# pinellolab/GRAFIMO

Hardware: AMD Instinct MI355X
Metric: scored haplotype k-mers/sec (higher is better)
Workload: dtype int32

## Files before the change

grafimo_amd/csrc/gfm_score_kernels.hpp:

```cpp
#pragma once

#include "gfm_common.hpp"

namespace {

constexpr int kWave = 64;
constexpr int kThreads = 1024;
constexpr int kWavesPerWG = kThreads / kWave;
constexpr unsigned kPoison = 0xFFFFu;
constexpr int kMaxLdsBytes = 160 * 1024;
constexpr int kWGsPerCU = 1;
constexpr int kReserveCUs = 4;
constexpr int kHitQueue = 64;

constexpr int kWorkspaces = GFM_WORKSPACE_RING;
constexpr int kCtlSlots = 2 * GFM_WORKSPACE_RING;
constexpr int kCtlAhead = GFM_WORKSPACE_RING;
struct HitCtl {
    unsigned long long mid[kCtlSlots];
    unsigned long long snap[kCtlSlots];
};
constexpr int kResidPerWG = kWavesPerWG * kHitQueue;

__device__ inline void hitq_push(long long *hitq, int &qn, bool hit, long long entry, int lane,
// ... 7 lines not shown
        unsigned long long base = 0;
        if (lane == 0) base = (hit_count ? *hit_count : 0ull) + atomicAdd(mid, (unsigned long long)qn);
        base = __shfl(base, 0);
        for (int i = lane; i < qn; i += kWave)
            if ((long long)(base + i) < hit_cap) hit_rows[base + i] = hitq[i];
        qn = 0;
    }
    if (hit) hitq[qn + __popcll(mask & ((1ull << lane) - 1ull))] = entry;
    qn += nh;
}

template <int WAVES>
__device__ inline void hitq_finish(const long long *hitq, int qn, int *wq_n ,
                                   int wave, int lane, int tid, long long *resid, int *resid_n)
{
    if (lane == 0) wq_n[wave] = qn;
    __syncthreads();
    int base = 0, tot = 0;
#pragma unroll
    for (int w = 0; w < WAVES; ++w) {
        if (w < wave) base += wq_n[w];
        tot += wq_n[w];
    }
    long long *slab = resid + (size_t)blockIdx.x * kResidPerWG;
    for (int i = lane; i < qn; i += kWave) slab[base + i] = hitq[i];
    if (tid == 0) resid_n[blockIdx.x] = tot;
}

constexpr int kSpillCopies = 16;

struct MotifArgs {
    const uint16_t *tab;
    int lo, nb, min_val;
    int use_hist;
    int spill_lo;
    int spill_n;
    unsigned *spill;
    int cutoff;
    int slot;
    int *scores;
    unsigned *partials;
    long long *hit_rows;
    long long hit_cap;
    const unsigned long long *hit_count;
    HitCtl *ctl;
    long long *resid;
    int *resid_n;
};
template <int MM> struct ScoreArgs {
    MotifArgs m[MM];
    int store_through;
};

typedef __attribute__((address_space(3))) const unsigned lds_cu32;
typedef __attribute__((address_space(3))) const uint16_t lds_cu16;
typedef __attribute__((address_space(3))) const unsigned long long lds_cu64;
__device__ inline unsigned lds_offset(const void *p)
{
    return (unsigned)(size_t)(__attribute__((address_space(3))) const char *)p;
}

constexpr int kSlabsPerGroup = 16;
constexpr int kPostJobs = 3;
struct PostJob {
    const unsigned *partials;
    unsigned long long *hist64;
    unsigned *spill;
    const long long *resid;
    const int *resid_n;
    HitCtl *ctl;
    long long *hit_rows;
    unsigned long long *hit_count;
    long long hit_cap;
    int nslabs, nb, lo, min_val, bin_blocks, hist_blocks, spill_lo, spill_n, spill_blocks, hit_slabs, par, total;
};
struct PostJobs { PostJob j[kPostJobs]; };

__device__ inline void
post_body(const unsigned *__restrict__ partials, int nslabs, int nb, int lo, int min_val,
          unsigned long long *__restrict__ hist64, int bin_blocks, int hist_blocks,
          unsigned *__restrict__ spill, int spill_lo, int spill_n, int spill_blocks,
          const long long *__restrict__ resid, const int *__restrict__ resid_n, int hit_slabs,
          HitCtl *__restrict__ ctl, int par, long long *__restrict__ hit_rows, long long hit_cap,
          unsigned long long *__restrict__ hit_count)
{
    const int tid = threadIdx.x;
    if (blockIdx.x == 0 && tid == 0 && hit_slabs == 0 && ctl) ctl->mid[(par + kCtlAhead) % kCtlSlots] = 0ull;
    if ((int)blockIdx.x < hist_blocks) {
        const int bx = blockIdx.x % bin_blocks, by = blockIdx.x / bin_blocks;
        const int b = bx * 256 + tid;
        if (b > nb) return;
        const int g0 = by * kSlabsPerGroup;
        const int g1 = min(g0 + kSlabsPerGroup, nslabs);
        unsigned long long s = 0;
        const size_t stride = (size_t)(nb + 1);
#pragma unroll 8
        for (int g = g0; g < g1; ++g) s += __builtin_nontemporal_load(&partials[g * stride + b]);
        if (s) atomicAdd(&hist64[b == nb ? min_val : lo + b], s);
        return;
    }
    if ((int)blockIdx.x < hist_blocks + spill_blocks) {
        const int b = ((int)blockIdx.x - hist_blocks) * 256 + tid;
        if (b < spill_n) {
            unsigned long long v = 0;
#pragma unroll
            for (int c = 0; c < kSpillCopies; ++c) {
                const unsigned x = spill[(size_t)c * (size_t)spill_n + b];
                if (x) {
                    v += x;
                    spill[(size_t)c * (size_t)spill_n + b] = 0u;
                }
            }
            if (v) atomicAdd(&hist64[spill_lo + b], v);
        }
        return;
    }
    __shared__ int part[256];
    __shared__ int part_all[256];
    const int g = blockIdx.x - hist_blocks - spill_blocks;
    int s = 0, sa = 0;
    for (int k = tid; k < hit_slabs; k += 256) {
        const int v = resid_n[k];
        sa += v;
        if (k < g) s += v;
    }
    part[tid] = s;
    part_all[tid] = sa;
    __syncthreads();
    for (int d = 128; d > 0; d >>= 1) {
        if (tid < d) { part[tid] += part[tid + d]; part_all[tid] += part_all[tid + d]; }
        __syncthreads();
    }
    const unsigned long long start = ctl->snap[par] + ctl->mid[par];
    const unsigned long long base = start + (unsigned long long)part[0];
    const int cnt = resid_n[g];
    const long long *slab = resid + (size_t)g * kResidPerWG;
    for (int i = tid; i < cnt; i += 256)
        if ((long long)(base + i) < hit_cap) __builtin_nontemporal_store(__builtin_nontemporal_load(&slab[i]), &hit_rows[base + i]);
    if (g == 0 && tid == 0) {
        *hit_count = start + (unsigned long long)part_all[0];
        ctl->mid[(par + kCtlAhead) % kCtlSlots] = 0ull;
    }
}

__global__ void __launch_bounds__(256) post_kernel(const PostJobs jobs)
{
    const PostJob &q = jobs.j[blockIdx.y];
    if ((int)blockIdx.x >= q.total) return;
    post_body(q.partials, q.nslabs, q.nb, q.lo, q.min_val, q.hist64, q.bin_blocks, q.hist_blocks, q.spill, q.spill_lo,
              q.spill_n, q.spill_blocks, q.resid, q.resid_n, q.hit_slabs, q.ctl, q.par, q.hit_rows, q.hit_cap,
              q.hit_count);
}

constexpr int kSelThreads = 256;
__global__ void __launch_bounds__(kSelThreads)
select_hits_kernel(const int *__restrict__ scores, long long n, const int *__restrict__ cutoff_ptr,
                   long long row_base, long long *__restrict__ hit_rows, long long hit_cap,
                   const unsigned long long *__restrict__ hit_count, HitCtl *__restrict__ ctl,
                   int par, long long *__restrict__ resid, int *__restrict__ resid_n,
                   const unsigned long long *__restrict__ gate_count, long long gate_cap)
{
    __shared__ long long hq[kSelThreads / kWave][kHitQueue];
    __shared__ int wq_n[kSelThreads / kWave];
    const int cutoff = *cutoff_ptr;
    const int tid = threadIdx.x, lane = tid & 63, wave = tid >> 6;
    long long *hitq = hq[wave];
    int qn = 0;
    if (gate_count) {
        if ((long long)*gate_count <= gate_cap) {
            if (tid == 0) {
                resid_n[blockIdx.x] = 0;
                if (blockIdx.x == 0) ctl->snap[par] = hit_count ? *hit_count : 0ull;
            }
            return;
        }
        hit_count = nullptr;
    }
    if (blockIdx.x == 0 && tid == 0) ctl->snap[par] = hit_count ? *hit_count : 0ull;
    const long long nthreads = (long long)gridDim.x * blockDim.x;
    const long long n4 = (n + 3) >> 2;
    const long long iters = (n4 + nthreads - 1) / nthreads;
    const long long t0 = (long long)blockIdx.x * blockDim.x + tid;
// ... 75 lines not shown
```

grafimo_amd/csrc/gfm_score_quad.hpp:

```cpp
#pragma once

#include "gfm_score_kernels.hpp"
#include "gfm_quad_launch.hpp"

namespace {

typedef unsigned u32x2_t __attribute__((ext_vector_type(2)));
typedef unsigned u32x4_t __attribute__((ext_vector_type(4)));
typedef __attribute__((address_space(3))) const u32x2_t lds_cu32x2;
typedef __attribute__((address_space(3))) const u32x4_t lds_cu32x4;
typedef int i32x4 __attribute__((ext_vector_type(4)));

template <int W, int MM, bool STORE = true>
__global__ void __launch_bounds__(kThreads)
score_quad_kernel(const uint8_t *__restrict__ kmers, long long n, long long row_base, const ScoreArgs<MM> a)
{
    extern __shared__ __attribute__((aligned(16))) unsigned char smem[];
    constexpr int NDW = (W + 3) / 4;
    constexpr int kTabBytes = quad_tab_bytes(W, MM);
    constexpr int CB = kQuadRows * W;
    constexpr int kLoads = (CB + 1023) / 1024;
    constexpr int GP = quad_pitch(W);
    constexpr int PAD = quad_pad(W);
    constexpr int SSTRIDE = quad_strip_stride(W, MM);

    if (lds_offset(smem) != 0u) __builtin_trap();
    const int tid = threadIdx.x;
    const int lane = tid & (kWave - 1);
    const int wave = __builtin_amdgcn_readfirstlane(tid >> 6);
    const int n_waves = (int)(blockDim.x >> 6);
    const int wg_threads = (int)blockDim.x;
    unsigned char *tab = smem;
    unsigned char *stage_base = smem + kTabBytes;
    unsigned *hist[MM];
    {
        unsigned *h = reinterpret_cast<unsigned *>(stage_base + n_waves * SSTRIDE);
#pragma unroll
        for (int m = 0; m < MM; ++m) {
            hist[m] = h;
            if (a.m[m].use_hist) h += a.m[m].nb + 1;
        }
    }

    unsigned char *stage = stage_base + wave * SSTRIDE;
    const unsigned stage_off = (unsigned)(kTabBytes + wave * SSTRIDE);
    const long long nfull = n / kQuadRows;
    const long long cstride = (long long)gridDim.x * n_waves;
    bool vec_store = true;
    const bool through = a.store_through == 1;
    constexpr bool no_store = !STORE;
#pragma unroll
    for (int m = 0; m < MM; ++m) vec_store = vec_store && (reinterpret_cast<uintptr_t>(a.m[m].scores) & 15u) == 0;

    uint4 pre[kQuadDepth][kLoads];
    auto fetch = [&](uint4 (&dst)[kLoads], long long c) {
        const uint8_t *src = kmers + c * (long long)CB + lane * 16;
#pragma unroll
        for (int i = 0; i < kLoads; ++i) {
            if (i * 1024 + 1024 <= CB || i * 1024 + lane * 16 < CB) {
                typedef unsigned u32x4 __attribute__((ext_vector_type(4)));
                const u32x4 t = __builtin_nontemporal_load(reinterpret_cast<const u32x4 *>(src + i * 1024));
                dst[i] = make_uint4(t.x, t.y, t.z, t.w);
            }
        }
    };

    long long *hitq[MM];
    int qn[MM];
    bool select[MM];
#pragma unroll
    for (int m = 0; m < MM; ++m) {
        hitq[m] = reinterpret_cast<long long *>(stage + quad_stage_bytes(W)) + m * kHitQueue;
        qn[m] = 0;
        select[m] = a.m[m].cutoff != GFM_NO_SELECT;
        if (select[m] && blockIdx.x == 0 && tid == 0)
            a.m[m].ctl->snap[a.m[m].slot] = a.m[m].hit_count ? *a.m[m].hit_count : 0ull;
    }

    int p_score[MM][4];
    long long p_crow = -1;
    auto book = [&]() {
        const int k0 = 4 * lane;
#pragma unroll
        for (int m = 0; m < MM; ++m) {
            const MotifArgs &ma = a.m[m];
            if (ma.use_hist) {
#pragma unroll
                for (int j = 0; j < 4; ++j) {
                    const unsigned off = (unsigned)(p_score[m][j] - ma.lo);
                    if (off < (unsigned)ma.nb)
                        atomicAdd(&hist[m][off], 1u);
                    else if (p_score[m][j] == ma.min_val)
                        atomicAdd(&hist[m][ma.nb], 1u);
                    else
                        atomicAdd(&ma.spill[(size_t)(blockIdx.x & (kSpillCopies - 1)) * (size_t)ma.spill_n + (size_t)(p_score[m][j] - ma.spill_lo)], 1u);
                }
            }
            if (select[m]) {
                const int best = max(max(p_score[m][0], p_score[m][1]), max(p_score[m][2], p_score[m][3]));
                if (__builtin_amdgcn_ballot_w64(best >= ma.cutoff)) {
#pragma unroll
                    for (int j = 0; j < 4; ++j)
                        hitq_push(hitq[m], qn[m], p_score[m][j] >= ma.cutoff,
                                  ((row_base + p_crow + k0 + j) << GFM_HIT_SCORE_BITS) | (long long)p_score[m][j], lane,
                                  ma.hit_count, &ma.ctl->mid[ma.slot], ma.hit_rows, ma.hit_cap);
                }
            }
        }
    };

    long long c = (long long)blockIdx.x * n_waves + wave;
#pragma unroll
    for (int d = 0; d < kQuadDepth; ++d)
        if (c + d * cstride < nfull) fetch(pre[d], c + d * cstride);
    if constexpr (MM == 1) {
        for (int i = tid; i < kTabBytes / 2; i += wg_threads) reinterpret_cast<uint16_t *>(tab)[i] = a.m[0].tab[i];
    } else {
        for (int i = tid; i < kTabBytes / 8; i += wg_threads) {
            unsigned long long v = 0;
            if (a.m[0].tab[i] == kPoison) {
                v = 1ull << 57;
            } else {
#pragma unroll
                for (int m = 0; m < MM; ++m) v |= (unsigned long long)a.m[m].tab[i] << (19 * m);
            }
            reinterpret_cast<unsigned long long *>(tab)[i] = v;
        }
    }
#pragma unroll
    for (int m = 0; m < MM; ++m)
        if (a.m[m].use_hist)
            for (int i = tid; i <= a.m[m].nb; i += wg_threads) hist[m][i] = 0u;
    __syncthreads();

    while (c < nfull) {
#pragma unroll
        for (int d = 0; d < kQuadDepth; ++d) {
            if (c >= nfull) break;
            const long long crow = c * kQuadRows;
            if (p_crow >= 0) book();
#pragma unroll
            for (int i = 0; i < kLoads; ++i) {
                const int off = i * 1024 + lane * 16;
                if (i * 1024 + 1024 <= CB || off < CB) {
                    const int dst = PAD ? off + PAD * (off / (4 * W)) : off;
                    *reinterpret_cast<uint4 *>(stage + dst) = pre[d][i];
                }
            }
            if (c + kQuadDepth * cstride < nfull) fetch(pre[d], c + kQuadDepth * cstride);
            __builtin_amdgcn_fence(__ATOMIC_RELEASE, "wavefront");
            __builtin_amdgcn_wave_barrier();

            unsigned w[W + 1];
            {
                const unsigned base = stage_off + (unsigned)(lane * GP);
                if constexpr (W % 2 == 1) {
#pragma unroll
                    for (int t = 0; t < W; ++t) w[t] = ((lds_cu32 *)(uintptr_t)base)[t];
                } else if constexpr (W % 4 == 2) {
#pragma unroll
                    for (int t = 0; t < W / 2; ++t) {
                        const u32x2_t v = ((lds_cu32x2 *)(uintptr_t)base)[t];
                        w[2 * t] = v.x;
                        w[2 * t + 1] = v.y;
                    }
                } else {
#pragma unroll
                    for (int t = 0; t < W / 4; ++t) {
                        const u32x4_t v = ((lds_cu32x4 *)(uintptr_t)base)[t];
                        w[4 * t] = v.x;
                        w[4 * t + 1] = v.y;
                        w[4 * t + 2] = v.z;
                        w[4 * t + 3] = v.w;
                    }
                }
                w[W] = 0u;
            }
            int score[MM][4];
#pragma unroll
            for (int j = 0; j < 4; ++j) {
                const int r = (j * W) & 3;
// ... 10 lines not shown
                        const unsigned e0 = y & 0x7Eu;
                        const unsigned e1 = (y >> 16) & 0x7Eu;
                        s1 += *(lds_cu16 *)(uintptr_t)(e0 + (unsigned)((2 * t) * 128));
                        s1 += *(lds_cu16 *)(uintptr_t)(e1 + (unsigned)((2 * t + 1) * 128));
                    }
                    any_n = (unsigned)s1 >= kPoison;
                    acc[0] = s1;
                } else {
                    unsigned long long s64 = 0;
#pragma unroll
                    for (int t = 0; t < NDW; ++t) {
                        const int q = (j * W + 4 * t) >> 2;
                        const unsigned x = r ? __builtin_amdgcn_alignbit(w[q + 1], w[q], (unsigned)(8 * r)) : w[q];
                        unsigned y;
                        asm("v_bfi_b32 %0, %1, %2, %3" : "=v"(y) : "s"(0x000E000Eu), "v"(x), "v"(x >> 5));
                        const unsigned e0 = (y & 0x7Eu) << 2;
                        const unsigned e1 = ((y >> 16) & 0x7Eu) << 2;
                        s64 += *(lds_cu64 *)(uintptr_t)(e0 + (unsigned)((2 * t) * 512));
                        s64 += *(lds_cu64 *)(uintptr_t)(e1 + (unsigned)((2 * t + 1) * 512));
                    }
                    any_n = (s64 >> 57) != 0;
#pragma unroll
                    for (int m = 0; m < MM; ++m) acc[m] = (int)((s64 >> (19 * m)) & 0x7FFFFull);
                }
#pragma unroll
                for (int m = 0; m < MM; ++m) score[m][j] = any_n ? a.m[m].min_val : acc[m];
            }
            const int k0 = 4 * lane;
#pragma unroll
            for (int m = 0; m < MM; ++m) {
                const __amdgpu_buffer_rsrc_t rs =
                    __builtin_amdgcn_make_buffer_rsrc(a.m[m].scores + crow, 0, kQuadRows * 4, 0x00020000);
                if (no_store) {
                } else if (vec_store) {
                    const u32x4_t out = {(unsigned)score[m][0], (unsigned)score[m][1], (unsigned)score[m][2],
                                         (unsigned)score[m][3]};
                    if (through)
                        __builtin_amdgcn_raw_buffer_store_b128(out, rs, k0 * 4, 0, kStoreThrough);
                    else
                        __builtin_amdgcn_raw_buffer_store_b128(out, rs, k0 * 4, 0, kStoreStream);
                } else {
#pragma unroll
                    for (int j = 0; j < 4; ++j) {
                        if (through)
                            __builtin_amdgcn_raw_buffer_store_b32((unsigned)score[m][j], rs, (k0 + j) * 4, 0, kStoreThrough);
                        else
                            __builtin_amdgcn_raw_buffer_store_b32((unsigned)score[m][j], rs, (k0 + j) * 4, 0, kStoreStream);
                    }
                }
#pragma unroll
                for (int j = 0; j < 4; ++j) p_score[m][j] = score[m][j];
            }
            p_crow = crow;
            __builtin_amdgcn_fence(__ATOMIC_ACQUIRE, "wavefront");
            __builtin_amdgcn_wave_barrier();
            c += cstride;
        }
    }
    if (p_crow >= 0) book();
    if (blockIdx.x == gridDim.x - 1 && wave == n_waves - 1 && nfull * kQuadRows < n) {
        const long long first = nfull * kQuadRows;
        const int count = (int)(n - first);
#pragma unroll 1
        for (int r0 = 0; r0 < count; r0 += kWave) {
            const int k = r0 + lane;
            const bool live = k < count;
            const uint8_t *row = kmers + (first + (live ? k : 0)) * (long long)W;
            unsigned long long s64 = 0;
            bool bad = false;
#pragma unroll 1
            for (int p = 0; p < 2 * NDW; ++p) {
                const unsigned b0 = 2 * p < W ? row[2 * p] : (unsigned)'A';
                const unsigned b1 = 2 * p + 1 < W ? row[2 * p + 1] : (unsigned)'A';
                const unsigned e = p * 64 + ((b0 >> 1) & 7u) + 8u * ((b1 >> 1) & 7u);
                if constexpr (MM == 1) {
                    const unsigned v = reinterpret_cast<const uint16_t *>(tab)[e];
                    bad = bad || v == kPoison;
                    s64 += v;
                } else {
                    s64 += reinterpret_cast<const unsigned long long *>(tab)[e];
                }
            }
            if constexpr (MM > 1) bad = (s64 >> 57) != 0;
#pragma unroll
            for (int m = 0; m < MM; ++m) {
                const MotifArgs &ma = a.m[m];
                const int sc = bad ? ma.min_val : (int)((MM == 1 ? s64 : (s64 >> (19 * m))) & 0x7FFFFull);
                if (live) {
                    if (!no_store) ma.scores[first + k] = sc;
                    if (ma.use_hist) {
                        const unsigned off = (unsigned)(sc - ma.lo);
                        if (off < (unsigned)ma.nb)
                            atomicAdd(&hist[m][off], 1u);
                        else if (sc == ma.min_val)
                            atomicAdd(&hist[m][ma.nb], 1u);
                        else
                            atomicAdd(&ma.spill[(size_t)(blockIdx.x & (kSpillCopies - 1)) * (size_t)ma.spill_n + (size_t)(sc - ma.spill_lo)], 1u);
                    }
                }
                if (select[m])
                    hitq_push(hitq[m], qn[m], live && sc >= ma.cutoff,
                              ((row_base + first + k) << GFM_HIT_SCORE_BITS) | (long long)sc, lane, ma.hit_count,
                              &ma.ctl->mid[ma.slot], ma.hit_rows, ma.hit_cap);
            }
        }
    }

    __syncthreads();
#pragma unroll
    for (int m = 0; m < MM; ++m) {
        const MotifArgs &ma = a.m[m];
        if (select[m]) {
            int *wq_n = reinterpret_cast<int *>(tab) + m * kWavesPerWG;
            if (lane == 0) wq_n[wave] = qn[m];
            __syncthreads();
            int base = 0, tot = 0;
            for (int w2 = 0; w2 < n_waves; ++w2) {
                const int v = wq_n[w2];
                if (w2 < wave) base += v;
                tot += v;
            }
            long long *slab = ma.resid + (size_t)blockIdx.x * kResidPerWG;
            for (int i = lane; i < qn[m]; i += kWave) slab[base + i] = hitq[m][i];
            if (tid == 0) ma.resid_n[blockIdx.x] = tot;
        }
        if (ma.use_hist) {
            unsigned *slab = ma.partials + (size_t)blockIdx.x * (size_t)(ma.nb + 1);
            for (int i = tid; i <= ma.nb; i += wg_threads) slab[i] = hist[m][i];
        }
    }
}

}
```

grafimo_amd/csrc/gfm_stats_kernels.hpp:

```cpp
#pragma once

#include "gfm_common.hpp"

namespace {

struct DpJob {
    long long sm;
    long long cum;
    long long bg;
    int W, L, lo, hi;
    double *buf;
    double *pmf;
    double *ptable;
};

constexpr int kDpThreads = 1024;

__global__ void __launch_bounds__(kDpThreads)
pvalue_dp_kernel(const DpJob *__restrict__ jobs, const int *__restrict__ ints, const double *__restrict__ dbls)
{
    const DpJob job = jobs[blockIdx.x];
    const int W = job.W, L = job.L;
    const int *__restrict__ sm = ints + job.sm;
    const int *__restrict__ cum_lo = ints + job.cum;
// ... 244 lines not shown
    int *cutoff;
    unsigned long long *nrows;
    unsigned long long *clear;
    int L, lo, hi, min_val, nblk;
};
struct QJobs {
    QJob j[kQJobs];
    double threshold;
    int on_qvalue;
};

__global__ void __launch_bounds__(kQThreads) q_count_kernel(const QJobs jobs)
{
    const QJob &q = jobs.j[blockIdx.y];
    if ((int)blockIdx.x >= q.nblk) return;
    q_count_body(q.hist, q.L, q.lo, q.hi, q.min_val, q.ws, q.cutoff);
}

__global__ void __launch_bounds__(kQThreads) q_raw_kernel(const QJobs jobs)
{
    const QJob &q = jobs.j[blockIdx.y];
    if ((int)blockIdx.x >= q.nblk) return;
    q_raw_body(q.hist, q.ptable, q.lo, q.hi, q.ws, q.qtable, q.nblk);
}

__global__ void __launch_bounds__(kQThreads) q_final_kernel(const QJobs jobs)
{
    const QJob &q = jobs.j[blockIdx.y];
    if ((int)blockIdx.x >= q.nblk) return;
    q_final_body(q.hist, q.ptable, q.L, q.lo, q.hi, q.min_val, jobs.threshold, jobs.on_qvalue, q.ws, q.qtable,
                 q.cutoff, q.nrows, q.clear, q.nblk);
}

}
```

grafimo_amd/csrc/grafimo_hip.hip:

```cpp

#include <hip/hip_runtime.h>

#include <algorithm>
#include <atomic>
#include <cmath>
#include <cstdarg>
#include <cstdint>
#include <cstdio>
#include <cstdlib>
#include <cstring>
#include <new>
#include <string>
#include <vector>

#include "grafimo_hip.h"

#define GFM_API extern "C" __attribute__((visibility("default")))

#include "gfm_hit_sort.hpp"
#include "gfm_common.hpp"
#include "gfm_score_kernels.hpp"
#include "gfm_quad_launch.hpp"
#include "gfm_stats_kernels.hpp"

// ... 183 lines not shown
    if (const char *e = std::getenv("GRAFIMO_STORE_POLICY")) {
        if (!std::strcmp(e, "through")) return 1;
        if (!std::strcmp(e, "stream")) return 0;
    }
#endif
    return n * 4ll * mm <= kStoreThroughMaxBytes ? 1 : 0;
}

size_t quad_fixed_lds(int W, int waves, int mm = 1)
{
    return (size_t)quad_tab_bytes(W, mm) + (size_t)waves * (size_t)quad_strip_stride(W, mm);
}

gfm_motif::Window best_window(gfm_motif *m, int bins)
{
    if (bins >= m->nb) return {m->nb, m->lo, 1.0};
    for (const auto &w : m->windows)
        if (w.bins == bins) return w;
    gfm_motif::Window best{bins, m->lo, -1.0};
    for (int a = m->lo; a + bins - 1 <= m->hi; ++a) {
        const int e = a + bins;
        const double mass = m->h_ptable[a] - (e < m->L ? m->h_ptable[e] : 0.0);
        if (mass > best.mass) { best.mass = mass; best.lo = a; }
    }
    m->windows.push_back(best);
    return best;
}

PostJob post_job(gfm_motif *m, const unsigned *partials, int hist_slabs, unsigned long long *d_hist,
                 int win_lo, int win_nb, unsigned *spill, const long long *resid, const int *resid_n, int hit_slabs,
                 HitCtl *ctl, int ctl_slot, long long *d_hit_rows, long long cap, unsigned long long *d_hit_count)
{
    PostJob q{};
    q.bin_blocks = (win_nb + 1 + 255) / 256;
    const int groups = (hist_slabs + kSlabsPerGroup - 1) / kSlabsPerGroup;
    q.hist_blocks = d_hist ? q.bin_blocks * groups : 0;
    q.spill_blocks = (d_hist && spill && win_nb < m->nb) ? (m->nb + 255) / 256 : 0;
    q.total = q.hist_blocks + q.spill_blocks + hit_slabs;
    q.partials = partials; q.hist64 = d_hist; q.spill = spill; q.resid = resid; q.resid_n = resid_n; q.ctl = ctl;
    q.hit_rows = d_hit_rows; q.hit_count = d_hit_count; q.hit_cap = cap;
    q.nslabs = hist_slabs; q.nb = win_nb; q.lo = win_lo; q.min_val = m->min_val;
    q.spill_lo = m->lo; q.spill_n = m->nb; q.hit_slabs = hit_slabs; q.par = ctl_slot;
    return q;
}

int launch_posts(const PostJob *jobs, int count, hipStream_t st)
{
    PostJobs all{};
    int live = 0, max_total = 0;
    for (int k = 0; k < count; ++k) {
        const PostJob &q = jobs[k];
        if (q.total == 0) {
            if (q.ctl)
                HIP_TRY(hipMemsetAsync(&q.ctl->mid[(q.par + kCtlAhead) % kCtlSlots], 0, sizeof(unsigned long long), st));
            continue;
        }
        all.j[live++] = q;
        max_total = std::max(max_total, q.total);
    }
    if (live == 0) return GFM_OK;
    hipLaunchKernelGGL(post_kernel, dim3((unsigned)max_total, (unsigned)live), dim3(256), 0, st, all);
    HIP_TRY(hipGetLastError());
    return GFM_OK;
}

int launch_post(gfm_motif *m, const unsigned *partials, int hist_slabs, unsigned long long *d_hist,
                int win_lo, int win_nb, unsigned *spill, const long long *resid, const int *resid_n, int hit_slabs, HitCtl *ctl, int ctl_slot,
                long long *d_hit_rows, long long cap, unsigned long long *d_hit_count, hipStream_t st)
{
    const PostJob q = post_job(m, partials, hist_slabs, d_hist, win_lo, win_nb, spill, resid, resid_n, hit_slabs, ctl,
                               ctl_slot, d_hit_rows, cap, d_hit_count);
    return launch_posts(&q, 1, st);
}

void fill_motif_args(MotifArgs &a, gfm_motif *m, int ws, int slot, int use_hist, int win_lo, int win_nb,
                     int cutoff,
                     int *d_scores, long long *d_hit_rows, long long cap,
                     const unsigned long long *d_hit_count_or_null)
{
    a.tab = m->d_tab;
    a.lo = win_lo;
    a.nb = win_nb;
    a.min_val = m->min_val;
    a.use_hist = use_hist;
    a.spill_lo = m->lo;
    a.spill_n = m->nb;
    a.spill = m->d_spill[ws];
    a.cutoff = cutoff;
    a.slot = slot;
    a.scores = d_scores;
    a.partials = m->d_partials[ws];
    a.hit_rows = d_hit_rows;
    a.hit_cap = cap;
    a.hit_count = d_hit_count_or_null;
    a.ctl = m->d_ctl;
    a.resid = m->d_resid[ws];
    a.resid_n = m->d_resid_n[ws];
}

bool plan_group(const gfm_motif_t *motifs, int n_left, const bool *with_hist, int *mm_out, int *waves_out,
                int *win_lo, int *win_nb)
{
    constexpr double kMinWindowMass = 0.999;
    const int W = motifs[0]->W;
    int mm = std::min(W <= kQuadMaxBatchWidth ? 3 : 1, n_left);
    int waves = kWavesPerWG;
    bool found = false;
    for (; mm >= 1 && !found; --mm) {
        for (int pass = mm > 1 ? 0 : 1; pass < 2 && !found; ++pass) {
            for (waves = kWavesPerWG; waves >= kWavesPerWG / 2 && !found; waves /= 2) {
                const long long spare = (long long)kMaxLdsBytes - (long long)quad_fixed_lds(W, waves, mm);
                long long room = spare / (long long)sizeof(unsigned);
                bool open[3] = {false, false, false};
                int users = 0;
                for (int k = 0; k < mm; ++k) {
// ... 212 lines not shown
            for (int c0 = 0; c0 < 8; ++c0) {
                bool bad = false;
                const unsigned v = base_score(2 * pr, c0, &bad) + base_score(2 * pr + 1, c1, &bad);
                tab[(size_t)pr * 64 + c0 + 8 * c1] = (uint16_t)(bad ? kPoison : v);
            }
    long long room16, room8;
    score_rooms(W, &room16, &room8);
    if (room8 < 256) return fail(GFM_ERR_INVALID, "no LDS left for a histogram window at width %d", W);
    m->part_nb = (int)std::min<long long>(m->nb, std::max(room16, room8));
    m->max_slabs = m->n_cu * kWGsPerCU;
    m->sel_slabs = 4 * m->n_cu;

    size_t slab_bytes = 0;
    auto carve = [&](size_t bytes) { const size_t at = slab_bytes; slab_bytes += align256(bytes); return at; };
    const size_t o_tab = carve(tab.size() * sizeof(uint16_t));
    ftab.assign((size_t)W * 8, 0u);
    {
        static const int row_of_code[4] = {0, 1, 3, 2};
        for (int j = 0; j < W; ++j)
            for (int c = 0; c < 4; ++c) {
                const unsigned fwd = (unsigned)sm[(size_t)row_of_code[c] * W + j];
                const unsigned rc_ = (unsigned)sm[(size_t)row_of_code[c ^ 2] * W + (W - 1 - j)];
                ftab[(size_t)j * 8 + c] = fwd | (rc_ << 16);
            }
    }
    const size_t o_ftab = carve(ftab.size() * sizeof(unsigned));
    const size_t o_pmf = carve(sizeof(double) * (size_t)m->L);
    const size_t o_ptable = carve(sizeof(double) * (size_t)m->L);
    const size_t o_dp = carve(sizeof(double) * 2 * (size_t)m->L);
    const size_t o_qwork = carve(sizeof(QWork) * kQStreams);
    const size_t o_qscratch = carve(sizeof(double) * (size_t)m->L * kQStreams);
    size_t o_partials[kWorkspaces], o_resid[kWorkspaces], o_resid_n[kWorkspaces], o_spill[kWorkspaces];
    for (int i = 0; i < kWorkspaces; ++i) {
        o_partials[i] = carve(sizeof(unsigned) * (size_t)m->max_slabs * (size_t)(m->part_nb + 1));
        o_resid[i] = carve(sizeof(long long) * (size_t)m->max_slabs * kResidPerWG);
        o_resid_n[i] = carve(sizeof(int) * (size_t)m->max_slabs);
    }
    const size_t o_sel_resid = carve(sizeof(long long) * (size_t)m->sel_slabs * kResidPerWG);
    const size_t o_sel_resid_n = carve(sizeof(int) * (size_t)m->sel_slabs);
    const size_t o_zero = slab_bytes;
    for (int i = 0; i < kWorkspaces; ++i) o_spill[i] = carve(sizeof(unsigned) * (size_t)m->nb * (size_t)kSpillCopies);
    const size_t o_ctl = carve(sizeof(HitCtl));
    const size_t o_sel_ctl = carve(sizeof(HitCtl));
    HIP_TRY(hipMalloc(&m->d_slab, slab_bytes));
    HIP_TRY(hipMemsetAsync(m->d_slab + o_zero, 0, slab_bytes - o_zero, nullptr));
    m->d_tab = reinterpret_cast<uint16_t *>(m->d_slab + o_tab);
    m->d_ftab = reinterpret_cast<unsigned *>(m->d_slab + o_ftab);
    m->d_pmf = reinterpret_cast<double *>(m->d_slab + o_pmf);
    m->d_ptable = reinterpret_cast<double *>(m->d_slab + o_ptable);
    m->d_qwork = reinterpret_cast<QWork *>(m->d_slab + o_qwork);
    m->d_qscratch = reinterpret_cast<double *>(m->d_slab + o_qscratch);
    for (int i = 0; i < kWorkspaces; ++i) {
        m->d_partials[i] = reinterpret_cast<unsigned *>(m->d_slab + o_partials[i]);
        m->d_resid[i] = reinterpret_cast<long long *>(m->d_slab + o_resid[i]);
        m->d_resid_n[i] = reinterpret_cast<int *>(m->d_slab + o_resid_n[i]);
        m->d_spill[i] = reinterpret_cast<unsigned *>(m->d_slab + o_spill[i]);
        HIP_TRY(hipEventCreateWithFlags(&m->ev_scored[i], hipEventDisableTiming | hipEventReleaseToDevice));
        HIP_TRY(hipEventCreateWithFlags(&m->ev_posted[i], hipEventDisableTiming | hipEventReleaseToDevice));
    }
    HIP_TRY(hipEventCreateWithFlags(&m->ev_selected, hipEventDisableTiming));
    m->d_sel_resid = reinterpret_cast<long long *>(m->d_slab + o_sel_resid);
    m->d_sel_resid_n = reinterpret_cast<int *>(m->d_slab + o_sel_resid_n);
    m->d_ctl = reinterpret_cast<HitCtl *>(m->d_slab + o_ctl);
    m->d_sel_ctl = reinterpret_cast<HitCtl *>(m->d_slab + o_sel_ctl);
    *d_rows = reinterpret_cast<double *>(m->d_slab + o_dp);

    HIP_TRY(hipMemcpyAsync(m->d_tab, tab.data(), tab.size() * sizeof(uint16_t), hipMemcpyHostToDevice, nullptr));
// ... 508 lines not shown
{
    if (!m || !n_out || (!h_ms && capacity)) return fail(GFM_ERR_INVALID, "NULL argument");
    const int used = std::min((int)m->tail_order.size(), capacity);
    for (int i = 0; i < used; ++i) {
        const int slot = m->tail_order[(size_t)i];
        HIP_TRY(hipEventSynchronize(m->tev1[slot]));
        HIP_TRY(hipEventElapsedTime(&h_ms[i], m->tev0[slot], m->tev1[slot]));
    }
    *n_out = used;
    m->tail_order.clear();
    return GFM_OK;
}

GFM_API int gfm_profile_read(gfm_motif_t m, float *h_ms, int capacity, int *n_out)
{
    if (!m || !n_out || (!h_ms && capacity)) return fail(GFM_ERR_INVALID, "NULL argument");
    const int slots = (int)m->ev0.size();
    const int used = std::min(m->ev_used, capacity);
    for (int i = 0; i < used; ++i) {
        const int slot = ((m->ev_next - m->ev_used + i) % slots + slots) % slots;
        HIP_TRY(hipEventSynchronize(m->ev1[slot]));
        HIP_TRY(hipEventElapsedTime(&h_ms[i], m->ev0[slot], m->ev1[slot]));
    }
    *n_out = used;
    m->ev_used = 0;
    return GFM_OK;
}

namespace {
int launch_qtables(const gfm_motif_t *motifs, int count, uint64_t *const *d_hist, double threshold, int on_qvalue,
                   double *const *d_qtable, int32_t *const *d_cutoff, uint64_t *const *d_nrows, uint32_t flags,
                   hipStream_t st)
{
    QJobs jobs{};
    jobs.threshold = threshold;
    jobs.on_qvalue = on_qvalue;
    int max_blk = 0;
    for (int k = 0; k < count; ++k) {
        gfm_motif *m = motifs[k];
        QJob &q = jobs.j[k];
        q.hist = reinterpret_cast<const unsigned long long *>(d_hist[k]);
        q.ptable = m->d_ptable;
        int qs = 0;
        while (qs < m->q_streams_used && m->q_stream[qs] != st) ++qs;
        if (qs == m->q_streams_used) {
            if (qs < kQStreams) {
                ++m->q_streams_used;
            } else {
                qs = 0;
                for (int c = 1; c < kQStreams; ++c)
                    if (m->q_last_use[c] < m->q_last_use[qs]) qs = c;
            }
            m->q_stream[qs] = st;
        }
        m->q_last_use[qs] = ++m->q_calls;
        q.ws = m->d_qwork + qs;
        q.qtable = (d_qtable && d_qtable[k]) ? d_qtable[k] : m->d_qscratch + (size_t)qs * (size_t)m->L;
        q.cutoff = d_cutoff ? d_cutoff[k] : nullptr;
        q.nrows = d_nrows ? reinterpret_cast<unsigned long long *>(d_nrows[k]) : nullptr;
        q.clear = (flags & GFM_FLAG_CLEAR_HIST) ? reinterpret_cast<unsigned long long *>(d_hist[k]) : nullptr;
        q.L = m->L; q.lo = m->lo; q.hi = m->hi; q.min_val = m->min_val;
        q.nblk = (m->nb + kQThreads - 1) / kQThreads;
        max_blk = std::max(max_blk, q.nblk);
    }
    const dim3 grid((unsigned)max_blk, (unsigned)count);
    hipLaunchKernelGGL(q_count_kernel, grid, dim3(kQThreads), 0, st, jobs);
    hipLaunchKernelGGL(q_raw_kernel, grid, dim3(kQThreads), 0, st, jobs);
    hipLaunchKernelGGL(q_final_kernel, grid, dim3(kQThreads), 0, st, jobs);
    HIP_TRY(hipGetLastError());
    return GFM_OK;
}
}

GFM_API int gfm_qvalue_table(gfm_motif_t m, uint64_t *d_hist, double threshold, int on_qvalue,
                             double *d_qtable, int32_t *d_cutoff, uint64_t *d_nrows, uint32_t flags,
                             void *stream)
{
    if (!m || !d_hist) return fail(GFM_ERR_INVALID, "NULL argument");
    return launch_qtables(&m, 1, &d_hist, threshold, on_qvalue, &d_qtable, &d_cutoff, &d_nrows, flags,
                          static_cast<hipStream_t>(stream));
}

GFM_API int gfm_qvalue_table_multi(const gfm_motif_t *motifs, int n_motifs, uint64_t *const *d_hist,
                                   double threshold, int on_qvalue, double *const *d_qtable,
                                   int32_t *const *d_cutoff, uint64_t *const *d_nrows, uint32_t flags, void *stream)
{
    if (!motifs || n_motifs < 1 || !d_hist) return fail(GFM_ERR_INVALID, "NULL argument");
    for (int i = 0; i < n_motifs; ++i) {
        if (!motifs[i] || !d_hist[i]) return fail(GFM_ERR_INVALID, "motif or histogram %d is NULL", i);
        for (int j = 0; j < i; ++j)
            if (motifs[j] == motifs[i]) return fail(GFM_ERR_INVALID, "motif %d listed twice", i);
    }
    for (int i = 0; i < n_motifs; i += kQJobs) {
        const int count = std::min(kQJobs, n_motifs - i);
        const int rc = launch_qtables(motifs + i, count, d_hist + i, threshold, on_qvalue,
                                      d_qtable ? d_qtable + i : nullptr, d_cutoff ? d_cutoff + i : nullptr,
                                      d_nrows ? d_nrows + i : nullptr, flags, static_cast<hipStream_t>(stream));
        if (rc) return rc;
    }
    return GFM_OK;
}
// ... 216 lines not shown
```

grafimo_amd/csrc/score_quad_tu.hip:

```cpp
#include <hip/hip_runtime.h>
#include <hip/hip_ext.h>

#include <atomic>
#include <cstdint>
#include <cstdio>
#include <string>

#include "grafimo_hip.h"

#include "gfm_common.hpp"
#include "gfm_score_quad.hpp"

#if !defined(GFM_QUAD_GROUP) || !defined(GFM_QUAD_MM)
#error "compile with -DGFM_QUAD_GROUP=0..3 -DGFM_QUAD_MM=1..3"
#endif

extern "C" void gfm_set_error_(const char *msg);

namespace {

int qfail(int code, const std::string &msg)
{
    gfm_set_error_(msg.c_str());
    return code;
}
#define Q_TRY(expr)                                                                            \
    do {                                                                                       \
        hipError_t e_ = (expr);                                                                \
        if (e_ != hipSuccess) return qfail(GFM_ERR_HIP, std::string(#expr " failed: ") + hipGetErrorString(e_)); \
    } while (0)

template <int W, int MM, bool STORE>
int launch_quad_k(const uint8_t *d_kmers, long long n, long long row_base, const ScoreArgs<MM> &args, size_t lds,
                  int nslabs, int waves, hipStream_t st, bool prepare, hipEvent_t ev0, hipEvent_t ev1)
{
    auto kern = score_quad_kernel<W, MM, STORE>;
    if (prepare) {
        static std::atomic<unsigned long long> done{0ull};
        int dev = 0;
        Q_TRY(hipGetDevice(&dev));
        const unsigned long long bit = 1ull << (dev & 63);
        if (done.load(std::memory_order_acquire) & bit) return GFM_OK;
        Q_TRY(hipFuncSetAttribute(reinterpret_cast<const void *>(kern), hipFuncAttributeMaxDynamicSharedMemorySize,
                                  kMaxLdsBytes));
        hipFuncAttributes attr;
        Q_TRY(hipFuncGetAttributes(&attr, reinterpret_cast<const void *>(kern)));
        if (attr.sharedSizeBytes != 0) return qfail(GFM_ERR_HIP, "score kernel carries static LDS (expected none)");
        done.fetch_or(bit, std::memory_order_release);
        return GFM_OK;
    }
    if (ev0 || ev1)
        hipExtLaunchKernelGGL(kern, dim3(nslabs), dim3(waves * kWave), lds, st, ev0, ev1, 0, d_kmers, n, row_base, args);
    else
        hipLaunchKernelGGL(kern, dim3(nslabs), dim3(waves * kWave), lds, st, d_kmers, n, row_base, args);
    Q_TRY(hipGetLastError());
    return GFM_OK;
}

template <int W, int MM>
int launch_quad_t(const uint8_t *d_kmers, long long n, long long row_base, const ScoreArgs<MM> &args, size_t lds,
                  int nslabs, int waves, hipStream_t st, bool prepare, hipEvent_t ev0, hipEvent_t ev1)
{
    if (prepare) {
        const int rc = launch_quad_k<W, MM, true>(d_kmers, n, row_base, args, lds, nslabs, waves, st, true, ev0, ev1);
        return rc ? rc : launch_quad_k<W, MM, false>(d_kmers, n, row_base, args, lds, nslabs, waves, st, true, ev0, ev1);
    }
    if (args.store_through == 2) return launch_quad_k<W, MM, false>(d_kmers, n, row_base, args, lds, nslabs, waves, st, false, ev0, ev1);
    return launch_quad_k<W, MM, true>(d_kmers, n, row_base, args, lds, nslabs, waves, st, false, ev0, ev1);
}

}

#define GFM_QUAD_NAME2(g, mm) gfm_quad_launch_g##g##_m##mm
#define GFM_QUAD_NAME(g, mm) GFM_QUAD_NAME2(g, mm)

extern "C" __attribute__((visibility("hidden"))) int GFM_QUAD_NAME(GFM_QUAD_GROUP, GFM_QUAD_MM)(
    int W, const uint8_t *d_kmers, long long n, long long row_base, const void *score_args, size_t lds, int nslabs,
    int waves, void *stream, int prepare, void *ev0, void *ev1)
{
    const ScoreArgs<GFM_QUAD_MM> &args = *static_cast<const ScoreArgs<GFM_QUAD_MM> *>(score_args);
    hipStream_t st = static_cast<hipStream_t>(stream);
    hipEvent_t e0 = static_cast<hipEvent_t>(ev0), e1 = static_cast<hipEvent_t>(ev1);
#define GFM_Q(N) case N: return launch_quad_t<N, GFM_QUAD_MM>(d_kmers, n, row_base, args, lds, nslabs, waves, st, prepare != 0, e0, e1);
    constexpr int B = 16 * GFM_QUAD_GROUP;
    switch (W) {
#ifdef GFM_ONLY_W
#if (GFM_ONLY_W - 1) / 16 == GFM_QUAD_GROUP
        GFM_Q(GFM_ONLY_W)
#endif
#else
        GFM_Q(B + 1) GFM_Q(B + 2) GFM_Q(B + 3) GFM_Q(B + 4) GFM_Q(B + 5) GFM_Q(B + 6) GFM_Q(B + 7) GFM_Q(B + 8)
        GFM_Q(B + 9) GFM_Q(B + 10) GFM_Q(B + 11) GFM_Q(B + 12) GFM_Q(B + 13) GFM_Q(B + 14) GFM_Q(B + 15) GFM_Q(B + 16)
#endif
        default: return qfail(GFM_ERR_INVALID, "unsupported width " + std::to_string(W));
    }
#undef GFM_Q
}
```

Baseline: 225.8 billion.

## Vectorize histogram reduction, specialize store forms, reorder staging, fuse q-value kernels

Partial histogram slabs are padded to a multiple of four bins so the post kernel can load them as 128-bit vectors, issuing all sixteen slab loads up front and summing four bins per thread. The score kernel picks its store variant (none, vector through, vector stream, scalar) at compile time instead of testing at runtime, and uses workgroup-scoped LDS atomics. It also moves the bookkeeping and the staging write for the next chunk to after the current chunk's stores, to change how work interleaves. For motifs with at most 8192 bins, the three-kernel q-value pass becomes one single-block kernel per motif. These changes add template instantiations and padding memory, and add a second q-value code path to maintain.

```diff
diff --git a/grafimo_amd/csrc/gfm_score_kernels.hpp b/grafimo_amd/csrc/gfm_score_kernels.hpp
--- a/grafimo_amd/csrc/gfm_score_kernels.hpp
+++ b/grafimo_amd/csrc/gfm_score_kernels.hpp
@@ -63,6 +63,7 @@
 struct MotifArgs {
     const uint16_t *tab;
     int lo, nb, min_val;
+    int slab_stride;
     int use_hist;
     int spill_lo;
     int spill_n;
@@ -84,6 +85,7 @@
 };
 
 typedef __attribute__((address_space(3))) const unsigned lds_cu32;
+typedef __attribute__((address_space(3))) unsigned lds_u32;
 typedef __attribute__((address_space(3))) const uint16_t lds_cu16;
 typedef __attribute__((address_space(3))) const unsigned long long lds_cu64;
 __device__ inline unsigned lds_offset(const void *p)
@@ -92,6 +94,7 @@
 }
 
 constexpr int kSlabsPerGroup = 16;
+__host__ __device__ constexpr int slab_stride_of(int nb) { return (nb + 1 + 3) & ~3; }
 constexpr int kPostJobs = 3;
 struct PostJob {
     const unsigned *partials;
@@ -103,12 +106,12 @@
     long long *hit_rows;
     unsigned long long *hit_count;
     long long hit_cap;
-    int nslabs, nb, lo, min_val, bin_blocks, hist_blocks, spill_lo, spill_n, spill_blocks, hit_slabs, par, total;
+    int nslabs, nb, slab_stride, lo, min_val, bin_blocks, hist_blocks, spill_lo, spill_n, spill_blocks, hit_slabs, par, total;
 };
 struct PostJobs { PostJob j[kPostJobs]; };
 
 __device__ inline void
-post_body(const unsigned *__restrict__ partials, int nslabs, int nb, int lo, int min_val,
+post_body(const unsigned *__restrict__ partials, int nslabs, int nb, int slab_stride, int lo, int min_val,
           unsigned long long *__restrict__ hist64, int bin_blocks, int hist_blocks,
           unsigned *__restrict__ spill, int spill_lo, int spill_n, int spill_blocks,
           const long long *__restrict__ resid, const int *__restrict__ resid_n, int hit_slabs,
@@ -119,15 +122,30 @@
     if (blockIdx.x == 0 && tid == 0 && hit_slabs == 0 && ctl) ctl->mid[(par + kCtlAhead) % kCtlSlots] = 0ull;
     if ((int)blockIdx.x < hist_blocks) {
         const int bx = blockIdx.x % bin_blocks, by = blockIdx.x / bin_blocks;
-        const int b = bx * 256 + tid;
-        if (b > nb) return;
+        const int b0 = 4 * (bx * 256 + tid);
+        if (b0 > nb) return;
         const int g0 = by * kSlabsPerGroup;
-        const int g1 = min(g0 + kSlabsPerGroup, nslabs);
-        unsigned long long s = 0;
-        const size_t stride = (size_t)(nb + 1);
-#pragma unroll 8
-        for (int g = g0; g < g1; ++g) s += __builtin_nontemporal_load(&partials[g * stride + b]);
-        if (s) atomicAdd(&hist64[b == nb ? min_val : lo + b], s);
+        typedef unsigned u32x4 __attribute__((ext_vector_type(4)));
+        const u32x4 *col = reinterpret_cast<const u32x4 *>(partials + b0);
+        const size_t stride4 = (size_t)(slab_stride >> 2);
+        u32x4 v[kSlabsPerGroup];
+#pragma unroll
+        for (int i = 0; i < kSlabsPerGroup; ++i)
+            v[i] = __builtin_nontemporal_load(&col[(size_t)min(g0 + i, nslabs - 1) * stride4]);
+        unsigned long long s[4] = {0ull, 0ull, 0ull, 0ull};
+#pragma unroll
+        for (int i = 0; i < kSlabsPerGroup; ++i)
+            if (g0 + i < nslabs) {
+                s[0] += v[i].x;
+                s[1] += v[i].y;
+                s[2] += v[i].z;
+                s[3] += v[i].w;
+            }
+#pragma unroll
+        for (int c = 0; c < 4; ++c) {
+            const int b = b0 + c;
+            if (b <= nb && s[c]) atomicAdd(&hist64[b == nb ? min_val : lo + b], s[c]);
+        }
         return;
     }
     if ((int)blockIdx.x < hist_blocks + spill_blocks) {
@@ -178,7 +196,7 @@
 {
     const PostJob &q = jobs.j[blockIdx.y];
     if ((int)blockIdx.x >= q.total) return;
-    post_body(q.partials, q.nslabs, q.nb, q.lo, q.min_val, q.hist64, q.bin_blocks, q.hist_blocks, q.spill, q.spill_lo,
+    post_body(q.partials, q.nslabs, q.nb, q.slab_stride, q.lo, q.min_val, q.hist64, q.bin_blocks, q.hist_blocks, q.spill, q.spill_lo,
               q.spill_n, q.spill_blocks, q.resid, q.resid_n, q.hit_slabs, q.ctl, q.par, q.hit_rows, q.hit_cap,
               q.hit_count);
 }
diff --git a/grafimo_amd/csrc/gfm_score_quad.hpp b/grafimo_amd/csrc/gfm_score_quad.hpp
--- a/grafimo_amd/csrc/gfm_score_quad.hpp
+++ b/grafimo_amd/csrc/gfm_score_quad.hpp
@@ -11,7 +11,8 @@
 typedef __attribute__((address_space(3))) const u32x4_t lds_cu32x4;
 typedef int i32x4 __attribute__((ext_vector_type(4)));
 
-template <int W, int MM, bool STORE = true>
+enum : int { kStoreNone = 0, kStoreVecThrough = 1, kStoreVecStream = 2, kStoreScalar = 3 };
+template <int W, int MM, int FORM = kStoreVecThrough>
 __global__ void __launch_bounds__(kThreads)
 score_quad_kernel(const uint8_t *__restrict__ kmers, long long n, long long row_base, const ScoreArgs<MM> a)
 {
@@ -33,24 +34,40 @@
     unsigned char *tab = smem;
     unsigned char *stage_base = smem + kTabBytes;
     unsigned *hist[MM];
+    unsigned hist_off[MM];
     {
         unsigned *h = reinterpret_cast<unsigned *>(stage_base + n_waves * SSTRIDE);
+        unsigned ho = (unsigned)(kTabBytes + n_waves * SSTRIDE);
 #pragma unroll
         for (int m = 0; m < MM; ++m) {
             hist[m] = h;
-            if (a.m[m].use_hist) h += a.m[m].nb + 1;
-        }
-    }
+            hist_off[m] = ho;
+            if (a.m[m].use_hist) {
+                h += a.m[m].nb + 1;
+                ho += 4u * (unsigned)(a.m[m].nb + 1);
+            }
+        }
+    }
+    auto count_row = [&](int m, int sc) __attribute__((always_inline)) {
+        const MotifArgs &ma = a.m[m];
+        const unsigned off = (unsigned)(sc - ma.lo);
+        if (off < (unsigned)ma.nb)
+            __hip_atomic_fetch_add((lds_u32 *)(uintptr_t)(hist_off[m] + 4u * off), 1u, __ATOMIC_RELAXED,
+                                   __HIP_MEMORY_SCOPE_WORKGROUP);
+        else if (sc == ma.min_val)
+            __hip_atomic_fetch_add((lds_u32 *)(uintptr_t)(hist_off[m] + 4u * (unsigned)ma.nb), 1u, __ATOMIC_RELAXED,
+                                   __HIP_MEMORY_SCOPE_WORKGROUP);
+        else
+            __hip_atomic_fetch_add(&ma.spill[(size_t)(blockIdx.x & (kSpillCopies - 1)) * (size_t)ma.spill_n + (size_t)(sc - ma.spill_lo)],
+                                   1u, __ATOMIC_RELAXED, __HIP_MEMORY_SCOPE_AGENT);
+    };
 
     unsigned char *stage = stage_base + wave * SSTRIDE;
     const unsigned stage_off = (unsigned)(kTabBytes + wave * SSTRIDE);
     const long long nfull = n / kQuadRows;
     const long long cstride = (long long)gridDim.x * n_waves;
-    bool vec_store = true;
     const bool through = a.store_through == 1;
-    constexpr bool no_store = !STORE;
-#pragma unroll
-    for (int m = 0; m < MM; ++m) vec_store = vec_store && (reinterpret_cast<uintptr_t>(a.m[m].scores) & 15u) == 0;
+    constexpr bool no_store = FORM == kStoreNone;
 
     uint4 pre[kQuadDepth][kLoads];
     auto fetch = [&](uint4 (&dst)[kLoads], long long c) {
@@ -79,22 +96,14 @@
 
     int p_score[MM][4];
     long long p_crow = -1;
-    auto book = [&]() {
+    auto book = [&]() __attribute__((always_inline)) {
         const int k0 = 4 * lane;
 #pragma unroll
         for (int m = 0; m < MM; ++m) {
             const MotifArgs &ma = a.m[m];
             if (ma.use_hist) {
 #pragma unroll
-                for (int j = 0; j < 4; ++j) {
-                    const unsigned off = (unsigned)(p_score[m][j] - ma.lo);
-                    if (off < (unsigned)ma.nb)
-                        atomicAdd(&hist[m][off], 1u);
-                    else if (p_score[m][j] == ma.min_val)
-                        atomicAdd(&hist[m][ma.nb], 1u);
-                    else
-                        atomicAdd(&ma.spill[(size_t)(blockIdx.x & (kSpillCopies - 1)) * (size_t)ma.spill_n + (size_t)(p_score[m][j] - ma.spill_lo)], 1u);
-                }
+                for (int j = 0; j < 4; ++j) count_row(m, p_score[m][j]);
             }
             if (select[m]) {
                 const int best = max(max(p_score[m][0], p_score[m][1]), max(p_score[m][2], p_score[m][3]));
@@ -133,20 +142,22 @@
             for (int i = tid; i <= a.m[m].nb; i += wg_threads) hist[m][i] = 0u;
     __syncthreads();
 
-    while (c < nfull) {
+    auto write_strip = [&](const uint4 (&src)[kLoads]) __attribute__((always_inline)) {
+#pragma unroll
+        for (int i = 0; i < kLoads; ++i) {
+            const int off = i * 1024 + lane * 16;
+            if (i * 1024 + 1024 <= CB || off < CB) {
+                const int dst = PAD ? off + PAD * (off / (4 * W)) : off;
+                *reinterpret_cast<uint4 *>(stage + dst) = src[i];
+            }
+        }
+    };
+    bool more = c < nfull;
+    if (more) write_strip(pre[0]);
+    while (more) {
 #pragma unroll
         for (int d = 0; d < kQuadDepth; ++d) {
-            if (c >= nfull) break;
             const long long crow = c * kQuadRows;
-            if (p_crow >= 0) book();
-#pragma unroll
-            for (int i = 0; i < kLoads; ++i) {
-                const int off = i * 1024 + lane * 16;
-                if (i * 1024 + 1024 <= CB || off < CB) {
-                    const int dst = PAD ? off + PAD * (off / (4 * W)) : off;
-                    *reinterpret_cast<uint4 *>(stage + dst) = pre[d][i];
-                }
-            }
             if (c + kQuadDepth * cstride < nfull) fetch(pre[d], c + kQuadDepth * cstride);
             __builtin_amdgcn_fence(__ATOMIC_RELEASE, "wavefront");
             __builtin_amdgcn_wave_barrier();
@@ -223,10 +234,10 @@
                 const __amdgpu_buffer_rsrc_t rs =
                     __builtin_amdgcn_make_buffer_rsrc(a.m[m].scores + crow, 0, kQuadRows * 4, 0x00020000);
                 if (no_store) {
-                } else if (vec_store) {
+                } else if constexpr (FORM != kStoreScalar) {
                     const u32x4_t out = {(unsigned)score[m][0], (unsigned)score[m][1], (unsigned)score[m][2],
                                          (unsigned)score[m][3]};
-                    if (through)
+                    if constexpr (FORM == kStoreVecThrough)
                         __builtin_amdgcn_raw_buffer_store_b128(out, rs, k0 * 4, 0, kStoreThrough);
                     else
                         __builtin_amdgcn_raw_buffer_store_b128(out, rs, k0 * 4, 0, kStoreStream);
@@ -246,6 +257,12 @@
             __builtin_amdgcn_fence(__ATOMIC_ACQUIRE, "wavefront");
             __builtin_amdgcn_wave_barrier();
             c += cstride;
+            if (c >= nfull) {
+                more = false;
+                break;
+            }
+            book();
+            write_strip(pre[(d + 1) % kQuadDepth]);
         }
     }
     if (p_crow >= 0) book();
@@ -279,15 +296,7 @@
                 const int sc = bad ? ma.min_val : (int)((MM == 1 ? s64 : (s64 >> (19 * m))) & 0x7FFFFull);
                 if (live) {
                     if (!no_store) ma.scores[first + k] = sc;
-                    if (ma.use_hist) {
-                        const unsigned off = (unsigned)(sc - ma.lo);
-                        if (off < (unsigned)ma.nb)
-                            atomicAdd(&hist[m][off], 1u);
-                        else if (sc == ma.min_val)
-                            atomicAdd(&hist[m][ma.nb], 1u);
-                        else
-                            atomicAdd(&ma.spill[(size_t)(blockIdx.x & (kSpillCopies - 1)) * (size_t)ma.spill_n + (size_t)(sc - ma.spill_lo)], 1u);
-                    }
+                    if (ma.use_hist) count_row(m, sc);
                 }
                 if (select[m])
                     hitq_push(hitq[m], qn[m], live && sc >= ma.cutoff,
@@ -316,8 +325,8 @@
             if (tid == 0) ma.resid_n[blockIdx.x] = tot;
         }
         if (ma.use_hist) {
-            unsigned *slab = ma.partials + (size_t)blockIdx.x * (size_t)(ma.nb + 1);
-            for (int i = tid; i <= ma.nb; i += wg_threads) slab[i] = hist[m][i];
+            unsigned *slab = ma.partials + (size_t)blockIdx.x * (size_t)ma.slab_stride;
+            for (int i = tid; i < ma.slab_stride; i += wg_threads) slab[i] = i <= ma.nb ? hist[m][i] : 0u;
         }
     }
 }
diff --git a/grafimo_amd/csrc/gfm_stats_kernels.hpp b/grafimo_amd/csrc/gfm_stats_kernels.hpp
--- a/grafimo_amd/csrc/gfm_stats_kernels.hpp
+++ b/grafimo_amd/csrc/gfm_stats_kernels.hpp
@@ -300,4 +300,106 @@
                  q.cutoff, q.nrows, q.clear, q.nblk);
 }
 
-}
+constexpr int kQFusedPer = 32;
+constexpr int kQFusedBins = kQThreads * kQFusedPer;
+
+__global__ void __launch_bounds__(kQThreads) q_fused_kernel(const QJobs jobs)
+{
+    const QJob &job = jobs.j[blockIdx.x];
+    const unsigned long long *hist = job.hist;
+    const double *__restrict__ ptable = job.ptable;
+    double *__restrict__ qtable = job.qtable;
+    const int L = job.L, lo = job.lo, hi = job.hi, min_val = job.min_val;
+    __shared__ unsigned long long sh[kQThreads / kWave];
+    __shared__ double shm[kQThreads / kWave];
+    __shared__ int first_s;
+    const int tid = threadIdx.x, lane = tid & 63, wave = tid >> 6;
+    const int j0 = lo + tid * kQFusedPer;
+    const bool n_outside = min_val < lo || min_val > hi;
+    if (tid == 0) first_s = L;
+
+    unsigned long long h[kQFusedPer];
+    double p[kQFusedPer];
+#pragma unroll
+    for (int i = 0; i < kQFusedPer; ++i) h[i] = hist[min(j0 + i, hi)];
+#pragma unroll
+    for (int i = 0; i < kQFusedPer; ++i) p[i] = ptable[min(j0 + i, hi)];
+    const unsigned long long n_rows_N = n_outside ? hist[min_val] : 0ull;
+    const double p_min_val = ptable[min_val];
+    unsigned long long mine = 0;
+#pragma unroll
+    for (int i = 0; i < kQFusedPer; ++i) {
+        if (j0 + i > hi) h[i] = 0ull;
+        mine += h[i];
+    }
+    unsigned long long cs = mine;
+#pragma unroll
+    for (int d = 1; d < kWave; d <<= 1) {
+        const unsigned long long v = __shfl_down(cs, d);
+        if (lane + d < kWave) cs += v;
+    }
+    if (lane == 0) sh[wave] = cs;
+    __syncthreads();
+    unsigned long long above = cs - mine, total = 0;
+#pragma unroll
+    for (int w = 0; w < kQThreads / kWave; ++w) {
+        if (w > wave) above += sh[w];
+        total += sh[w];
+    }
+    const unsigned long long n = total + n_rows_N;
+    const double nd = (double)n;
+    double tmin = INFINITY;
+    {
+        unsigned long long c_ge = above;
+#pragma unroll
+        for (int i = kQFusedPer - 1; i >= 0; --i) {
+            c_ge += h[i];
+            const double raw = h[i] ? p[i] / ((double)c_ge / nd) : INFINITY;
+            h[i] = (unsigned long long)__double_as_longlong(raw);
+            tmin = fmin(tmin, raw);
+        }
+    }
+    double ms = tmin;
+#pragma unroll
+    for (int d = 1; d < kWave; d <<= 1) {
+        const double v = __shfl_up(ms, d);
+        if (lane >= d) ms = fmin(ms, v);
+    }
+    if (lane == kWave - 1) shm[wave] = ms;
+    double below = __shfl_up(ms, 1);
+    if (lane == 0) below = INFINITY;
+    __syncthreads();
+    double all = INFINITY;
+#pragma unroll
+    for (int w = 0; w < kQThreads / kWave; ++w) {
+        if (w < wave) below = fmin(below, shm[w]);
+        all = fmin(all, shm[w]);
+    }
+    const double base = n_rows_N ? p_min_val / (nd / nd) : INFINITY;
+    double run = fmin(below, base);
+    int first = L;
+#pragma unroll
+    for (int i = 0; i < kQFusedPer; ++i) {
+        const int j = j0 + i;
+        run = fmin(run, __longlong_as_double((long long)h[i]));
+        const double q = fmin(run, 1.0);
+        if (j <= hi) {
+            qtable[j] = q;
+            const double val = jobs.on_qvalue ? q : p[i];
+            if (val < jobs.threshold) first = min(first, j);
+            if (job.clear) job.clear[j] = 0ull;
+        }
+    }
+    if (first < L) atomicMin(&first_s, first);
+    const double q_above = fmin(fmin(base, all), 1.0);
+    for (int jj = tid; jj < lo; jj += kQThreads) qtable[jj] = fmin(base, 1.0);
+    for (int jj = hi + 1 + tid; jj < L; jj += kQThreads) qtable[jj] = q_above;
+    __syncthreads();
+    if (tid == 0) {
+        if (job.cutoff) *job.cutoff = first_s;
+        if (job.nrows) *job.nrows = n;
+        if (job.clear && n_outside) job.clear[min_val] = 0ull;
+    }
+}
+
+}
diff --git a/grafimo_amd/csrc/grafimo_hip.hip b/grafimo_amd/csrc/grafimo_hip.hip
--- a/grafimo_amd/csrc/grafimo_hip.hip
+++ b/grafimo_amd/csrc/grafimo_hip.hip
@@ -239,7 +239,8 @@
                  HitCtl *ctl, int ctl_slot, long long *d_hit_rows, long long cap, unsigned long long *d_hit_count)
 {
     PostJob q{};
-    q.bin_blocks = (win_nb + 1 + 255) / 256;
+    q.slab_stride = slab_stride_of(win_nb);
+    q.bin_blocks = (q.slab_stride / 4 + 255) / 256;
     const int groups = (hist_slabs + kSlabsPerGroup - 1) / kSlabsPerGroup;
     q.hist_blocks = d_hist ? q.bin_blocks * groups : 0;
     q.spill_blocks = (d_hist && spill && win_nb < m->nb) ? (m->nb + 255) / 256 : 0;
@@ -288,6 +289,7 @@
     a.tab = m->d_tab;
     a.lo = win_lo;
     a.nb = win_nb;
+    a.slab_stride = slab_stride_of(win_nb);
     a.min_val = m->min_val;
     a.use_hist = use_hist;
     a.spill_lo = m->lo;
@@ -566,7 +568,7 @@
     const size_t o_qscratch = carve(sizeof(double) * (size_t)m->L * kQStreams);
     size_t o_partials[kWorkspaces], o_resid[kWorkspaces], o_resid_n[kWorkspaces], o_spill[kWorkspaces];
     for (int i = 0; i < kWorkspaces; ++i) {
-        o_partials[i] = carve(sizeof(unsigned) * (size_t)m->max_slabs * (size_t)(m->part_nb + 1));
+        o_partials[i] = carve(sizeof(unsigned) * (size_t)m->max_slabs * (size_t)slab_stride_of(m->part_nb));
         o_resid[i] = carve(sizeof(long long) * (size_t)m->max_slabs * kResidPerWG);
         o_resid_n[i] = carve(sizeof(int) * (size_t)m->max_slabs);
     }
@@ -1141,13 +1143,13 @@
                    double *const *d_qtable, int32_t *const *d_cutoff, uint64_t *const *d_nrows, uint32_t flags,
                    hipStream_t st)
 {
-    QJobs jobs{};
-    jobs.threshold = threshold;
-    jobs.on_qvalue = on_qvalue;
-    int max_blk = 0;
+    QJobs jobs{}, fused{};
+    jobs.threshold = fused.threshold = threshold;
+    jobs.on_qvalue = fused.on_qvalue = on_qvalue;
+    int max_blk = 0, n_wide = 0, n_fused = 0;
     for (int k = 0; k < count; ++k) {
         gfm_motif *m = motifs[k];
-        QJob &q = jobs.j[k];
+        QJob &q = m->nb <= kQFusedBins ? fused.j[n_fused++] : jobs.j[n_wide++];
         q.hist = reinterpret_cast<const unsigned long long *>(d_hist[k]);
         q.ptable = m->d_ptable;
         int qs = 0;
@@ -1170,12 +1172,15 @@
         q.clear = (flags & GFM_FLAG_CLEAR_HIST) ? reinterpret_cast<unsigned long long *>(d_hist[k]) : nullptr;
         q.L = m->L; q.lo = m->lo; q.hi = m->hi; q.min_val = m->min_val;
         q.nblk = (m->nb + kQThreads - 1) / kQThreads;
-        max_blk = std::max(max_blk, q.nblk);
-    }
-    const dim3 grid((unsigned)max_blk, (unsigned)count);
-    hipLaunchKernelGGL(q_count_kernel, grid, dim3(kQThreads), 0, st, jobs);
-    hipLaunchKernelGGL(q_raw_kernel, grid, dim3(kQThreads), 0, st, jobs);
-    hipLaunchKernelGGL(q_final_kernel, grid, dim3(kQThreads), 0, st, jobs);
+        if (m->nb > kQFusedBins) max_blk = std::max(max_blk, q.nblk);
+    }
+    if (n_fused > 0) hipLaunchKernelGGL(q_fused_kernel, dim3((unsigned)n_fused), dim3(kQThreads), 0, st, fused);
+    if (n_wide > 0) {
+        const dim3 grid((unsigned)max_blk, (unsigned)n_wide);
+        hipLaunchKernelGGL(q_count_kernel, grid, dim3(kQThreads), 0, st, jobs);
+        hipLaunchKernelGGL(q_raw_kernel, grid, dim3(kQThreads), 0, st, jobs);
+        hipLaunchKernelGGL(q_final_kernel, grid, dim3(kQThreads), 0, st, jobs);
+    }
     HIP_TRY(hipGetLastError());
     return GFM_OK;
 }
diff --git a/grafimo_amd/csrc/score_quad_tu.hip b/grafimo_amd/csrc/score_quad_tu.hip
--- a/grafimo_amd/csrc/score_quad_tu.hip
+++ b/grafimo_amd/csrc/score_quad_tu.hip
@@ -30,11 +30,11 @@
         if (e_ != hipSuccess) return qfail(GFM_ERR_HIP, std::string(#expr " failed: ") + hipGetErrorString(e_)); \
     } while (0)
 
-template <int W, int MM, bool STORE>
+template <int W, int MM, int FORM>
 int launch_quad_k(const uint8_t *d_kmers, long long n, long long row_base, const ScoreArgs<MM> &args, size_t lds,
                   int nslabs, int waves, hipStream_t st, bool prepare, hipEvent_t ev0, hipEvent_t ev1)
 {
-    auto kern = score_quad_kernel<W, MM, STORE>;
+    auto kern = score_quad_kernel<W, MM, FORM>;
     if (prepare) {
         static std::atomic<unsigned long long> done{0ull};
         int dev = 0;
@@ -61,12 +61,19 @@
 int launch_quad_t(const uint8_t *d_kmers, long long n, long long row_base, const ScoreArgs<MM> &args, size_t lds,
                   int nslabs, int waves, hipStream_t st, bool prepare, hipEvent_t ev0, hipEvent_t ev1)
 {
+#define GFM_QUAD_FORM(F) launch_quad_k<W, MM, F>(d_kmers, n, row_base, args, lds, nslabs, waves, st, prepare, ev0, ev1)
     if (prepare) {
-        const int rc = launch_quad_k<W, MM, true>(d_kmers, n, row_base, args, lds, nslabs, waves, st, true, ev0, ev1);
-        return rc ? rc : launch_quad_k<W, MM, false>(d_kmers, n, row_base, args, lds, nslabs, waves, st, true, ev0, ev1);
+        int rc = GFM_QUAD_FORM(kStoreNone);
+        if (!rc) rc = GFM_QUAD_FORM(kStoreVecThrough);
+        if (!rc) rc = GFM_QUAD_FORM(kStoreVecStream);
+        return rc ? rc : GFM_QUAD_FORM(kStoreScalar);
     }
-    if (args.store_through == 2) return launch_quad_k<W, MM, false>(d_kmers, n, row_base, args, lds, nslabs, waves, st, false, ev0, ev1);
-    return launch_quad_k<W, MM, true>(d_kmers, n, row_base, args, lds, nslabs, waves, st, false, ev0, ev1);
+    if (args.store_through == 2) return GFM_QUAD_FORM(kStoreNone);
+    bool vec = true;
+    for (int m = 0; m < MM; ++m) vec = vec && (reinterpret_cast<uintptr_t>(args.m[m].scores) & 15u) == 0;
+    if (!vec) return GFM_QUAD_FORM(kStoreScalar);
+    return args.store_through == 1 ? GFM_QUAD_FORM(kStoreVecThrough) : GFM_QUAD_FORM(kStoreVecStream);
+#undef GFM_QUAD_FORM
 }
 
 }
```

Result: slower. 214.1 billion (-5.2%).
